# mvrl/RANGE

Measured on AMD Instinct MI355X. Metric: geo-embeddings/sec (10k-query batch, range_db_large), higher is better.
Workload: dtype f32

## Files before the change

### range_amd/csrc/attend_kernels.h

```cpp
#pragma once
#include <hip/hip_runtime.h>
#include <stdint.h>

#include <type_traits>

#include "host_plan.h"

namespace range_hip {

typedef float f32x4 __attribute__((ext_vector_type(4)));

constexpr int KEY_DIM = 256;
constexpr int VAL_DIM = 1024;
constexpr int QTILE = 64;
constexpr int BLK = 16;
constexpr int MAX_TOPK = 16;
constexpr float NEG_BIG = -1.0e30f;

#define RANGE_LPTR(p) ((__attribute__((address_space(3))) void*)(p))

__device__ __forceinline__ int pi_row(int i) { return ((i & 2) << 2) | ((i >> 2) << 1) | (i & 1); }

struct ScanArgs {
    const float* keys;
// ... 307 lines not shown
            if (a.rowmax)
                smax = fmaxf(smax, fmaxf(fmaxf(ok[0] ? ss[0] : -INFINITY, ok[1] ? ss[1] : -INFINITY),
                                         fmaxf(ok[2] ? ss[2] : -INFINITY, ok[3] ? ss[3] : -INFINITY)));
#pragma unroll
            for (int r = 0; r < 4; ++r) {
                const float p1 = __builtin_amdgcn_exp2f(fmaf(ss[r], a.k_sem, nm1));
                l1 += ok[r] ? p1 : 0.f;
                if (GEO) {
                    const float p2 = __builtin_amdgcn_exp2f(fmaf(sg[r], a.k_geo, nm2));
                    l2 += ok[r] ? p2 : 0.f;
                }
            }
        };
        if (n_here == BLK) tile_stats(std::false_type{});
        else tile_stats(std::true_type{});
        slot ^= 1;
    }
#pragma unroll
    for (int off = 16; off <= 32; off <<= 1) {
        l1 += __shfl_xor(l1, off);
        if (GEO) l2 += __shfl_xor(l2, off);
    }
    const float m1 = a.k_sem;
    float m2 = a.k_geo;
    if (!GEO) { m2 = NEG_BIG; l2 = 0.f; }
    if (q < a.B) {
        if (a.rowmax) a.rowmax[((int64_t)split * a.B + q) * 4 + g] = smax;
        if (g == 0) {
            f32x4 o = {m1, l1, m2, l2};
            *reinterpret_cast<f32x4*>(a.out + ((int64_t)split * a.B + q) * 4) = o;
        }
        if (TOPK) {
            const int64_t base = (((int64_t)split * a.B + q) * 4 + g) * MAX_TOPK;
#pragma unroll
            for (int k = 0; k < MAX_TOPK; ++k) {
                a.cand_val[base + k] = tk.v[TOPK ? k : 0];
                a.cand_idx[base + k] = tk.i[TOPK ? k : 0];
            }
        }
    }
}

__device__ __forceinline__ unsigned long long topk_key(float v, uint32_t row) {
    const uint32_t b = __float_as_uint(v);
    const uint32_t o = (b & 0x80000000u) ? ~b : (b | 0x80000000u);
    return ((unsigned long long)o << 32) | (unsigned long long)(0xFFFFFFFFu - row);
}
__device__ __forceinline__ float topk_key_val(unsigned long long k) {
    const uint32_t o = (uint32_t)(k >> 32);
    return __uint_as_float((o & 0x80000000u) ? (o & 0x7FFFFFFFu) : ~o);
}
__device__ __forceinline__ uint32_t topk_key_row(unsigned long long k) { return 0xFFFFFFFFu - (uint32_t)k; }

struct KeyList {
    unsigned long long k[MAX_TOPK];
    __device__ __forceinline__ void init() {
#pragma unroll
        for (int i = 0; i < MAX_TOPK; ++i) k[i] = 0ull;
    }
    __device__ __forceinline__ void push(unsigned long long x) {
        if (x > k[MAX_TOPK - 1]) {
            k[MAX_TOPK - 1] = x;
#pragma unroll
            for (int i = MAX_TOPK - 1; i > 0; --i) {
                const unsigned long long a = k[i - 1], b = k[i];
                k[i - 1] = a > b ? a : b;
                k[i] = a > b ? b : a;
            }
        }
    }
    __device__ __forceinline__ void pop() {
#pragma unroll
        for (int i = 0; i + 1 < MAX_TOPK; ++i) k[i] = k[i + 1];
        k[MAX_TOPK - 1] = 0ull;
    }
};

typedef uint32_t range_u32x2 __attribute__((ext_vector_type(2)));
__device__ __forceinline__ uint32_t lane_xor16(uint32_t x) {
    const range_u32x2 r = __builtin_amdgcn_permlane16_swap(x, x, false, false);
    return (__lane_id() & 16) ? r[0] : r[1];
}
__device__ __forceinline__ uint32_t lane_xor32(uint32_t x) {
    const range_u32x2 r = __builtin_amdgcn_permlane32_swap(x, x, false, false);
    return (__lane_id() & 32) ? r[0] : r[1];
}
__device__ __forceinline__ float lane_xor16(float x) { return __uint_as_float(lane_xor16(__float_as_uint(x))); }
__device__ __forceinline__ float lane_xor32(float x) { return __uint_as_float(lane_xor32(__float_as_uint(x))); }

__device__ __forceinline__ unsigned long long shfl_xor_u64(unsigned long long x, int m) {
    const uint32_t lo = __shfl_xor((uint32_t)x, m), hi = __shfl_xor((uint32_t)(x >> 32), m);
    return ((unsigned long long)hi << 32) | lo;
}
template <int M>
__device__ __forceinline__ unsigned long long lane_xor_u64(unsigned long long x) {
    static_assert(M == 16 || M == 32, "row swaps exist for lane ^ 16 and lane ^ 32");
    const uint32_t lo = M == 16 ? lane_xor16((uint32_t)x) : lane_xor32((uint32_t)x);
    const uint32_t hi = M == 16 ? lane_xor16((uint32_t)(x >> 32)) : lane_xor32((uint32_t)(x >> 32));
    return ((unsigned long long)hi << 32) | lo;
}

__device__ __forceinline__ void merge_lane_groups(KeyList& L) {
    KeyList R;
#pragma unroll
    for (int i = 0; i < MAX_TOPK; ++i) {
        const unsigned long long h = L.k[0];
        unsigned long long m = h;
        unsigned long long o = lane_xor_u64<16>(m); m = o > m ? o : m;
        o = lane_xor_u64<32>(m); m = o > m ? o : m;
        R.k[i] = m;
        if (h == m && m != 0ull) L.pop();
    }
    L = R;
}

__device__ __forceinline__ void merge_wave(KeyList& L) {
    KeyList R;
#pragma unroll
    for (int i = 0; i < MAX_TOPK; ++i) {
        const unsigned long long h = L.k[0];
        unsigned long long m = h;
#pragma unroll
        for (int off = 1; off < 64; off <<= 1) {
            const unsigned long long o = shfl_xor_u64(m, off);
            m = o > m ? o : m;
        }
        R.k[i] = m;
        if (h == m && m != 0ull) L.pop();
    }
    L = R;
}

__global__ __launch_bounds__(256) void topk_threshold_kernel(const float* __restrict__ rowmax,
                                                             int n_parts, int64_t B,
                                                             float* __restrict__ theta) {
    const int lane = threadIdx.x & 63;
    const int64_t q = (int64_t)blockIdx.x * 4 + (threadIdx.x >> 6);
    if (q >= B) return;
    KeyList L;
    L.init();
    const int total = n_parts * 4;
    for (int e = lane; e < total; e += 64) {
        const float v = rowmax[((int64_t)(e >> 2) * B + q) * 4 + (e & 3)];
        if (v > -INFINITY) L.push(topk_key(v, (uint32_t)e));
    }
    merge_wave(L);
    if (lane == 0) theta[q] = L.k[MAX_TOPK - 1] ? topk_key_val(L.k[MAX_TOPK - 1]) : -INFINITY;
}

__global__ __launch_bounds__(256) void topk_from_logits_kernel(const float* __restrict__ logits,
                                                               int32_t n_blocks, int64_t B,
                                                               int64_t n_valid, int32_t n_chunks,
                                                               const float* __restrict__ theta,
                                                               float* __restrict__ cval,
                                                               int32_t* __restrict__ cidx) {
    const int lane = threadIdx.x & 63, g = lane >> 4;
    const int64_t slot = (int64_t)blockIdx.x * 4 + (threadIdx.x >> 6);
    const int64_t n_slots = (B + 15) / 16;
    if (slot >= n_slots) return;
    const int chunk = blockIdx.y;
    const int b0 = (int)(((int64_t)chunk * n_blocks) / n_chunks);
    const int b1 = (int)(((int64_t)(chunk + 1) * n_blocks) / n_chunks);
    const float* base = logits + ((slot >> 2) * (int64_t)n_blocks * 4 + (slot & 3)) * 256 + 4 * lane;
    int prow[4];
#pragma unroll
    for (int r = 0; r < 4; ++r) prow[r] = pi_row(4 * g + r);
    KeyList L;
    L.init();
    const int64_t qq = slot * 16 + (lane & 15);
    const float th = theta[qq < B ? qq : B - 1];
    constexpr int UNROLL = 8;
    for (int b = b0; b < b1; b += UNROLL) {
        f32x4 v[UNROLL];
#pragma unroll
        for (int u = 0; u < UNROLL; ++u) {
            const int bb = b + u < b1 ? b + u : b1 - 1;
            v[u] = *reinterpret_cast<const f32x4*>(base + (int64_t)bb * 1024);
        }
#pragma unroll
        for (int u = 0; u < UNROLL; ++u) {
            if (b + u < b1) {
                const int64_t row0 = (int64_t)(b + u) * BLK;
#pragma unroll
                for (int r = 0; r < 4; ++r) {
                    const int64_t row = row0 + prow[r];
                    if (v[u][r] >= th && row < n_valid) L.push(topk_key(v[u][r], (uint32_t)row));
                }
            }
        }
    }
    merge_lane_groups(L);
    const int64_t q = slot * 16 + (lane & 15);
    if (g == 0 && q < B) {
        float* ov = cval + ((int64_t)chunk * B + q) * MAX_TOPK;
        int32_t* oi = cidx + ((int64_t)chunk * B + q) * MAX_TOPK;
#pragma unroll
        for (int i = 0; i < MAX_TOPK; ++i) {
            const unsigned long long mm = L.k[i];
            ov[i] = mm ? topk_key_val(mm) : -INFINITY;
            oi[i] = mm ? (int32_t)topk_key_row(mm) : 0x7fffffff;
        }
    }
}

__global__ __launch_bounds__(256) void merge_topk_wave_kernel(const float* __restrict__ cval,
                                                              const int32_t* __restrict__ cidx,
                                                              int n_parts, int64_t B, int per_part,
                                                              int k, int64_t row_offset,
                                                              float* __restrict__ oval,
                                                              int64_t* __restrict__ oidx) {
    const int lane = threadIdx.x & 63;
    const int64_t q = (int64_t)blockIdx.x * 4 + (threadIdx.x >> 6);
    if (q >= B) return;
    KeyList L;
    L.init();
    const int total = n_parts * per_part;
    for (int e = lane; e < total; e += 64) {
        const int p = e / per_part, c = e - p * per_part;
        const int64_t at = ((int64_t)p * B + q) * per_part + c;
        const int32_t row = cidx[at];
        if (row != 0x7fffffff) L.push(topk_key(cval[at], (uint32_t)row));
    }
    merge_wave(L);
    if (lane == 0) {
#pragma unroll
        for (int i = 0; i < MAX_TOPK; ++i) {
            if (i < k) {
                const unsigned long long mm = L.k[i];
                oval[q * k + i] = mm ? topk_key_val(mm) : -INFINITY;
                oidx[q * k + i] = mm ? (int64_t)topk_key_row(mm) + row_offset : (int64_t)-1;
            }
        }
    }
}

__global__ void merge_stats_kernel(const float* parts, int n_parts, int64_t B, float* out) {
    const int64_t q = (int64_t)blockIdx.x * blockDim.x + threadIdx.x;
    if (q >= B) return;
    float m1 = NEG_BIG, l1 = 0.f, m2 = NEG_BIG, l2 = 0.f;
    for (int p = 0; p < n_parts; ++p) {
        const f32x4 s = *reinterpret_cast<const f32x4*>(parts + ((int64_t)p * B + q) * 4);
        merge_ml(m1, l1, s.x, s.y);
        merge_ml(m2, l2, s.z, s.w);
    }
    f32x4 o = {m1, l1, m2, l2};
    *reinterpret_cast<f32x4*>(out + q * 4) = o;
}

__global__ __launch_bounds__(256) void merge_stats_wave_kernel(const float* __restrict__ parts,
                                                               int n_parts, int64_t B,
                                                               float* __restrict__ out) {
    const int lane = threadIdx.x & 63;
    const int64_t q = (int64_t)blockIdx.x * 4 + (threadIdx.x >> 6);
    if (q >= B) return;
    float m1 = NEG_BIG, l1 = 0.f, m2 = NEG_BIG, l2 = 0.f;
    for (int p = lane; p < n_parts; p += 64) {
        const f32x4 s = *reinterpret_cast<const f32x4*>(parts + ((int64_t)p * B + q) * 4);
        merge_ml(m1, l1, s.x, s.y);
        merge_ml(m2, l2, s.z, s.w);
    }
#pragma unroll
    for (int off = 1; off < 64; off <<= 1) {
        merge_ml(m1, l1, __shfl_xor(m1, off), __shfl_xor(l1, off));
        merge_ml(m2, l2, __shfl_xor(m2, off), __shfl_xor(l2, off));
    }
    if (lane == 0) {
        f32x4 o = {m1, l1, m2, l2};
        *reinterpret_cast<f32x4*>(out + q * 4) = o;
    }
}

__global__ void merge_topk_kernel(const float* cval, const int32_t* cidx32, const int64_t* cidx64,
                                  int n_parts, int64_t B, int per_part, int k, int64_t row_offset,
                                  float* oval, int64_t* oidx) {
    const int64_t q = (int64_t)blockIdx.x * blockDim.x + threadIdx.x;
    if (q >= B) return;
    float bv[MAX_TOPK];
    int64_t bi[MAX_TOPK];
    for (int j = 0; j < MAX_TOPK; ++j) { bv[j] = -INFINITY; bi[j] = INT64_MAX; }
    for (int p = 0; p < n_parts; ++p) {
        const int64_t base = ((int64_t)p * B + q) * per_part;
        for (int c = 0; c < per_part; ++c) {
            const float v = cval[base + c];
            const int64_t i = cidx32 ? (cidx32[base + c] == 0x7fffffff
                                            ? INT64_MAX : (int64_t)cidx32[base + c] + row_offset)
                                     : cidx64[base + c];
            if (i == INT64_MAX) continue;
            if (v > bv[k - 1] || (v == bv[k - 1] && i < bi[k - 1])) {
                int j = k - 1;
                while (j > 0 && (v > bv[j - 1] || (v == bv[j - 1] && i < bi[j - 1]))) {
                    bv[j] = bv[j - 1]; bi[j] = bi[j - 1]; --j;
                }
                bv[j] = v; bi[j] = i;
            }
        }
    }
    for (int j = 0; j < k; ++j) { oval[q * k + j] = bv[j]; oidx[q * k + j] = bi[j] == INT64_MAX ? -1 : bi[j]; }
}

__device__ __forceinline__ void mfma_a(f32x4& acc, float a, float b) {
    asm volatile("v_mfma_f32_16x16x4_f32 %0, %1, %2, %0\n\ts_nop 1" : "+a"(acc) : "v"(a), "v"(b));
}

struct PvCarry {
    f32x4 v0a, v1a, v0b, v1b;
    float w0, w1;
};

struct PvOps { f32x4 v0, v1; };

__device__ __forceinline__ void pv_first_reads(const float* vslot, int lane, PvOps& s0, PvOps& s1) {
    const float* base = vslot + (2 * (lane >> 4)) * VAL_DIM + 4 * (lane & 15);
    s0.v0 = *reinterpret_cast<const f32x4*>(base);
    s0.v1 = *reinterpret_cast<const f32x4*>(base + VAL_DIM);
    s1.v0 = *reinterpret_cast<const f32x4*>(base + 64);
    s1.v1 = *reinterpret_cast<const f32x4*>(base + VAL_DIM + 64);
}

__device__ __forceinline__ void pv_exec_carry(f32x4 (&acc)[64], const PvCarry& c) {
    mfma_a(acc[56], c.w0, c.v0a.x);
    mfma_a(acc[57], c.w0, c.v0a.y);
    mfma_a(acc[58], c.w0, c.v0a.z);
    mfma_a(acc[59], c.w0, c.v0a.w);
    mfma_a(acc[56], c.w1, c.v1a.x);
    mfma_a(acc[57], c.w1, c.v1a.y);
    mfma_a(acc[58], c.w1, c.v1a.z);
    mfma_a(acc[59], c.w1, c.v1a.w);
    mfma_a(acc[60], c.w0, c.v0b.x);
    mfma_a(acc[61], c.w0, c.v0b.y);
    mfma_a(acc[62], c.w0, c.v0b.z);
    mfma_a(acc[63], c.w0, c.v0b.w);
    mfma_a(acc[60], c.w1, c.v1b.x);
    mfma_a(acc[61], c.w1, c.v1b.y);
    mfma_a(acc[62], c.w1, c.v1b.z);
    mfma_a(acc[63], c.w1, c.v1b.w);
}

#define RANGE_PV_MFMA(tile, w, v, h)                 \
    mfma_a(acc[tile], w, v);                         \
    __builtin_amdgcn_sched_barrier(0);               \
    hook(h);                                         \
    __builtin_amdgcn_sched_barrier(0)

template <class Hook>
__device__ __forceinline__ void pv_steps(const float* vslot, float w0, float w1, PvOps s0, PvOps s1,
                                         f32x4 (&acc)[64], int lane, PvCarry& carry, Hook&& hook) {
    const float* base = vslot + (2 * (lane >> 4)) * VAL_DIM + 4 * (lane & 15);
    f32x4 v0 = s0.v0, v1 = s0.v1, n0 = s1.v0, n1 = s1.v1;
#pragma unroll
    for (int T = 0; T < 14; ++T) {
        const f32x4 m0 = *reinterpret_cast<const f32x4*>(base + 64 * (T + 2));
        const f32x4 m1 = *reinterpret_cast<const f32x4*>(base + VAL_DIM + 64 * (T + 2));
        RANGE_PV_MFMA(4 * T + 0, w0, v0.x, 8 * T + 0);
        RANGE_PV_MFMA(4 * T + 1, w0, v0.y, 8 * T + 1);
        RANGE_PV_MFMA(4 * T + 2, w0, v0.z, 8 * T + 2);
        RANGE_PV_MFMA(4 * T + 3, w0, v0.w, 8 * T + 3);
        RANGE_PV_MFMA(4 * T + 0, w1, v1.x, 8 * T + 4);
        RANGE_PV_MFMA(4 * T + 1, w1, v1.y, 8 * T + 5);
        RANGE_PV_MFMA(4 * T + 2, w1, v1.z, 8 * T + 6);
        RANGE_PV_MFMA(4 * T + 3, w1, v1.w, 8 * T + 7);
        v0 = n0; v1 = n1; n0 = m0; n1 = m1;
    }
    carry.v0a = v0; carry.v1a = v1; carry.v0b = n0; carry.v1b = n1; carry.w0 = w0; carry.w1 = w1;
}
#undef RANGE_PV_MFMA

__device__ __forceinline__ void acc_fence(f32x4 (&acc)[64]) {
    asm volatile("s_nop 15\n\ts_nop 7" ::: "memory");
#pragma unroll
    for (int i = 0; i < 64; i += 16)
        asm volatile("" : "+a"(acc[i]), "+a"(acc[i + 1]), "+a"(acc[i + 2]), "+a"(acc[i + 3]),
                          "+a"(acc[i + 4]), "+a"(acc[i + 5]), "+a"(acc[i + 6]), "+a"(acc[i + 7]),
                          "+a"(acc[i + 8]), "+a"(acc[i + 9]), "+a"(acc[i + 10]), "+a"(acc[i + 11]),
                          "+a"(acc[i + 12]), "+a"(acc[i + 13]), "+a"(acc[i + 14]), "+a"(acc[i + 15]));
}

struct SegWalk {
    int64_t u, u_end;
    int split, col, cb0, cb;
    __device__ __forceinline__ void init(const ScanArgs& a) {
        col = -1;
        u = u_end = 0;
        cb0 = 0;
        cb = a.n_blocks;
        split = 0;
        if (a.sk_groups == 0) {
            int qt;
            decode_block(a, split, qt);
            const int b0 = (int)(((int64_t)split * a.n_blocks) / a.n_splits);
            const int b1 = (int)(((int64_t)(split + 1) * a.n_blocks) / a.n_splits);
            u = (int64_t)qt * a.n_blocks + b0;
            u_end = u + (b1 - b0);
        }
    }
    __device__ __forceinline__ bool next(const ScanArgs& a, int& qt, int& b0, int& b1, float*& out_tile) {
        if (a.sk_groups == 0) {
            if (u >= u_end) return false;
            qt = (int)(u / a.n_blocks);
            b0 = (int)(u - (int64_t)qt * a.n_blocks);
            b1 = b0 + (int)(u_end - u);
            out_tile = a.out + ((int64_t)split * a.B + (int64_t)qt * QTILE) * VAL_DIM;
            u = u_end;
            return true;
        }
        while (u >= u_end) {
            if (++col >= a.sk_cols) return false;
            cb0 = sk_col_begin(col, a.n_blocks, a.sk_cols);
            cb = sk_col_begin(col + 1, a.n_blocks, a.sk_cols) - cb0;
            const int64_t U = (int64_t)a.n_qtiles * cb;
            u = sk_start(blockIdx.x, U, a.sk_groups);
            u_end = sk_start((int64_t)blockIdx.x + 1, U, a.sk_groups);
        }
        qt = (int)(u / cb);
        const int bo = (int)(u - (int64_t)qt * cb);
        const int64_t left = u_end - u;
        const int n = left < (int64_t)(cb - bo) ? (int)left : cb - bo;
        b0 = cb0 + bo;
        b1 = b0 + n;
        out_tile = a.out + ((int64_t)col * (a.sk_groups + a.n_qtiles) + blockIdx.x + qt) * (QTILE * VAL_DIM);
        u += n;
        return true;
    }
};

constexpr int ATTEND_LDS_BYTES = (3 * 8 * VAL_DIM + 2 * BLK * KEY_DIM + 2 * 64) * 4;
constexpr int P1_WG_PER_CU = 4;
constexpr int SCAN_LDS_BYTES = (2 * BLK * KEY_DIM + 2 * 64) * 4;

template <bool GEO, bool DIAG = false>
__global__ __launch_bounds__(256, 1) void attend_kernel(ScanArgs a) {
    extern __shared__ __attribute__((aligned(16))) char smem[];
    float* vring = reinterpret_cast<float*>(smem);

    const uint32_t lds0 = (uint32_t)(uintptr_t)RANGE_LPTR(smem);
    const uint32_t vring_lds = lds0;
    const uint32_t kring_lds = lds0 + 3 * 8 * VAL_DIM * 4;
    const uint32_t xring_lds = kring_lds + 2 * BLK * KEY_DIM * 4;
    constexpr uint32_t VS_BYTES = 8 * VAL_DIM * 4, KT_BYTES = BLK * KEY_DIM * 4;

    const int lane = threadIdx.x & 63;
    const int wave = __builtin_amdgcn_readfirstlane(threadIdx.x >> 6);
    const int g = lane >> 4;
    const int swz = lane ^ (4 * wave);
    SegWalk walk;
    walk.init(a);
    int qt, b0, b1;
    float* out_tile;
    for (bool first_seg = true; walk.next(a, qt, b0, b1, out_tile); first_seg = false) {
    if (!first_seg) __syncthreads();
    const int nb = b1 - b0;
    const int64_t q = (int64_t)qt * QTILE + wave * 16 + (lane & 15);

    QFrag f;
    load_qfrag(f, a.ehat, a.xq, a.B, q, g);
    float ca, cb, m1, m2;
    {
        const f32x4 st = *reinterpret_cast<const f32x4*>(a.stats + (q < a.B ? q : a.B - 1) * 4);
        m1 = st.x; m2 = st.z;
        ca = a.beta / st.y;
        cb = GEO ? (1.0f - a.beta) / st.w : 0.f;
    }
    pin_qfrag(f);
    asm volatile("" : "+v"(ca), "+v"(cb), "+v"(m1), "+v"(m2));

    f32x4 acc[64];
#pragma unroll
    for (int i = 0; i < 64; ++i) acc[i] = f32x4{0.f, 0.f, 0.f, 0.f};

    KAddr kaddr;
    kaddr.init(lane);
    const char* kring_b = smem + 3 * 8 * VAL_DIM * 4;
    const char* xring_b = kring_b + 2 * BLK * KEY_DIM * 4;
    int prow[4];
    uint32_t kvoff[4];
#pragma unroll
    for (int r = 0; r < 4; ++r) {
        prow[r] = pi_row(4 * g + r);
        kvoff[r] = (uint32_t)((swz ^ r) << 4);
    }
    const int n_left = (int)(a.n_valid - (int64_t)b0 * BLK);

    f32x4 w_cur = {0.f, 0.f, 0.f, 0.f};
    if (nb > 0) {
        const int64_t r0 = (int64_t)b0 * BLK;
        const int64_t r1 = (int64_t)(nb > 1 ? b0 + 1 : b0) * BLK;
        issue_k_tile(a.keys, a.xyz4, r0, kring_lds, xring_lds, wave, lane, swz);
        issue_v_half(a.values, r0, vring_lds, wave, lane);
        issue_v_half(a.values, r0 + 8, vring_lds + VS_BYTES, wave, lane);
        issue_k_tile(a.keys, a.xyz4, r1, kring_lds + KT_BYTES, xring_lds + 256, wave, lane, swz);
        RANGE_WAIT_BARRIER(21);
        QKAcc c;
        qk_mfma<GEO>(kring_b, qk_first_reads<GEO>(kring_b, xring_b, kaddr), kaddr, f, c,
                     [](int) __attribute__((always_inline)) {});
        c.fence();
#pragma unroll
        for (int r = 0; r < 4; ++r) {
            float wr = ca * __builtin_amdgcn_exp2f(fmaf(c.sem(r), a.k_sem, -m1));
            if (GEO) wr = fmaf(cb, __builtin_amdgcn_exp2f(fmaf(c.g[r], a.k_geo, -m2)), wr);
            w_cur[r] = prow[r] < n_left ? wr : 0.f;
        }
    }
    int vs = 0;
    PvCarry carry;
    carry.v0a = carry.v1a = carry.v0b = carry.v1b = f32x4{0.f, 0.f, 0.f, 0.f};
    carry.w0 = carry.w1 = 0.f;
    unsigned long long d_vm0 = 0, d_bar0 = 0, d_pv0 = 0, d_vm1 = 0, d_bar1 = 0, d_qk = 0, d_pv1 = 0;
    unsigned long long d_mark = 0;
    const unsigned long long d_start = DIAG ? stamp() : 0;
    const int b_last = b1 - 1;
    for (int t = 0; t < nb; ++t) {
        const int vs1 = vs == 2 ? 0 : vs + 1;
        const int vs2 = vs1 == 2 ? 0 : vs1 + 1;
        const int bn1 = min(b0 + t + 1, b_last), bn2 = min(b0 + t + 2, b_last);
        const float* vsrc1 = a.values + ((int64_t)bn1 * BLK + 2 * wave) * VAL_DIM;
        const float* ksrc2 = a.keys + ((int64_t)bn2 * BLK + 4 * wave) * KEY_DIM;
        const float* xsrc2 = a.xyz4 + (int64_t)bn2 * BLK * 4;
        const uint32_t vdst_e = vring_lds + vs2 * VS_BYTES + wave * 8192;
        const uint32_t vdst_o = vring_lds + vs * VS_BYTES + wave * 8192;
        const uint32_t kdst = kring_lds + (t & 1) * KT_BYTES + wave * 4096;
        const uint32_t xdst = xring_lds + (t & 1) * 256;
        const uint32_t vvoff = (uint32_t)(lane << 4);
        RANGE_WB(13, d_vm0, d_bar0);
        if (DIAG) d_mark = stamp();
        {
            PvOps s0, s1;
            pv_first_reads(vring + vs * 8 * VAL_DIM, lane, s0, s1);
            pv_exec_carry(acc, carry);
            pv_steps(vring + vs * 8 * VAL_DIM, w_cur[0], w_cur[1], s0, s1, acc, lane, carry,
                     [&](int h) __attribute__((always_inline)) {
                         if (h % 14 == 3) {
                             const int ii = h / 14;
                             if ((ii & 3) == 0) dma_group_begin(vdst_e + (ii >> 2) * 4096);
                             dma_b128_q(vsrc1 + (ii >> 2) * VAL_DIM, vvoff, ii & 3);
                         }
                     });
        }
        if (DIAG) d_pv0 += stamp() - d_mark;
        RANGE_WB(8, d_vm1, d_bar1);
        if (DIAG) d_mark = stamp();
        QKAcc c;
        PvOps s0, s1;
        {
            const char* kt = kring_b + ((t + 1) & 1) * KT_BYTES;
            const KFirst kf = qk_first_reads<GEO>(kt, xring_b + ((t + 1) & 1) * 256, kaddr);
            pv_exec_carry(acc, carry);
            qk_mfma<GEO>(kt, kf, kaddr, f, c, [&](int s_) __attribute__((always_inline)) {
                if (s_ == 13) pv_first_reads(vring + vs1 * 8 * VAL_DIM, lane, s0, s1);
            });
        }
        if (DIAG) { const unsigned long long x_ = stamp(); d_qk += x_ - d_mark; d_mark = x_; }
        f32x4 w_next = {0.f, 0.f, 0.f, 0.f};
        float e1[4], e2[4];
        const int n_left1 = n_left - (t + 1) * BLK;
        pv_steps(vring + vs1 * 8 * VAL_DIM, w_cur[2], w_cur[3], s0, s1, acc, lane, carry,
                [&](int h) __attribute__((always_inline)) {
                    if ((h & 7) == 3) {
                        const int ii = h >> 3;
                        if (ii < 8) {
                            if ((ii & 3) == 0) dma_group_begin(vdst_o + (ii >> 2) * 4096);
                            dma_b128_q(vsrc1 + (8 + (ii >> 2)) * VAL_DIM, vvoff, ii & 3);
                        } else if (ii < 12) {
                            if (ii == 8) dma_group_begin(kdst);
                            dma_b128_q(ksrc2, kvoff[ii - 8], ii - 8);
                        } else if (ii == 12) {
                            dma_b32(xsrc2, (uint32_t)(lane << 2), xdst);
                        }
                    } else if (h >= 21 && h < 101 && ((h - 21) & 3) == 0) {
                        const int k = (h - 21) >> 2, r = k / 5, part = k % 5;
                        if (part == 0) {
                        } else if (part == 1) {
                            e1[r] = fmaf(c.a0[r], a.k_sem, -m1);
                            if (GEO) e2[r] = fmaf(c.g[r], a.k_geo, -m2);
                        } else if (part == 2) {
                            e1[r] = __builtin_amdgcn_exp2f(e1[r]);
                        } else if (part == 3) {
                            if (GEO) e2[r] = __builtin_amdgcn_exp2f(e2[r]);
                        } else {
                            float wr = ca * e1[r];
                            if (GEO) wr = fmaf(cb, e2[r], wr);
                            w_next[r] = prow[r] < n_left1 ? wr : 0.f;
                        }
                    }
                });
        if (DIAG) d_pv1 += stamp() - d_mark;
        w_cur = w_next;
        vs = vs2;
    }
    if (nb > 0) pv_exec_carry(acc, carry);
    asm volatile("s_waitcnt vmcnt(0)" ::: "memory");
    if (DIAG && lane == 0 && a.diag) {
        unsigned long long* d = a.diag + ((size_t)blockIdx.x * 4 + wave) * 16;
        d[0] = d_vm0; d[1] = d_bar0; d[2] = d_pv0; d[3] = d_vm1; d[4] = d_bar1; d[5] = d_qk;
        d[6] = d_pv1; d[7] = stamp() - d_start; d[8] = (unsigned long long)nb; d[9] = d_start;
        unsigned xcc; asm volatile("s_getreg_b32 %0, hwreg(HW_REG_XCC_ID)" : "=s"(xcc));
        d[10] = xcc & 0xf;
    }

    acc_fence(acc);
    const int j = lane & 15;
    const int64_t qw = (int64_t)qt * QTILE + wave * 16;
#pragma unroll
    for (int r = 0; r < 4; ++r) {
        const int64_t qo = qw + 4 * g + r;
        if (qo < a.B) {
            float* orow = out_tile + (wave * 16 + 4 * g + r) * VAL_DIM + 4 * j;
#pragma unroll
            for (int T = 0; T < 16; ++T) {
                f32x4 o = {acc[4 * T + 0][r], acc[4 * T + 1][r], acc[4 * T + 2][r], acc[4 * T + 3][r]};
                *reinterpret_cast<f32x4*>(orow + 64 * T) = o;
            }
        }
    }
    }
}

constexpr int ATTEND_STORED_LDS_BYTES = (3 * 8 * VAL_DIM + 2 * 1024 + 2 * 64) * 4;

template <bool GEO>
__global__ __launch_bounds__(256, 1) void attend_stored_kernel(ScanArgs a) {
    extern __shared__ __attribute__((aligned(16))) char smem[];
    float* vring = reinterpret_cast<float*>(smem);
    const uint32_t lds0 = (uint32_t)(uintptr_t)RANGE_LPTR(smem);
    const uint32_t vring_lds = lds0;
    const uint32_t sring_lds = lds0 + 3 * 8 * VAL_DIM * 4;
    const uint32_t xring_lds = sring_lds + 2 * 4096;
    constexpr uint32_t VS_BYTES = 8 * VAL_DIM * 4;

    const int lane = threadIdx.x & 63;
    const int wave = __builtin_amdgcn_readfirstlane(threadIdx.x >> 6);
    const int g = lane >> 4;
    SegWalk walk;
    walk.init(a);
    int qt, b0, b1;
    float* out_tile;
    for (bool first_seg = true; walk.next(a, qt, b0, b1, out_tile); first_seg = false) {
    if (!first_seg) __syncthreads();
    const int nb = b1 - b0;
    const int64_t q = (int64_t)qt * QTILE + wave * 16 + (lane & 15);
    const int64_t qtile_kept = (int64_t)qt + a.qt_offset;

    float ca, cb, m1, m2, fxq;
    {
        const int64_t qq = q < a.B ? q : a.B - 1;
        const f32x4 st = *reinterpret_cast<const f32x4*>(a.stats + qq * 4);
        m1 = st.x; m2 = st.z;
        ca = a.beta / st.y;
        cb = GEO ? (1.0f - a.beta) / st.w : 0.f;
        fxq = a.xq[qq * 4 + g];
    }
    asm volatile("" : "+v"(ca), "+v"(cb), "+v"(m1), "+v"(m2), "+v"(fxq));

    f32x4 acc[64];
#pragma unroll
    for (int i = 0; i < 64; ++i) acc[i] = f32x4{0.f, 0.f, 0.f, 0.f};

    const char* sring_b = smem + 3 * 8 * VAL_DIM * 4;
    const char* xring_b = sring_b + 2 * 4096;
    const uint32_t s_rd = (uint32_t)(wave * 1024 + lane * 16);
    const uint32_t x_rd = (uint32_t)((pi_row(lane & 15) * 4 + g) * 4);
    int prow[4];
#pragma unroll
    for (int r = 0; r < 4; ++r) prow[r] = pi_row(4 * g + r);
    const int n_left = (int)(a.n_valid - (int64_t)b0 * BLK);
    const uint32_t vvoff = (uint32_t)(lane << 4);

    auto issue_sx = [&](int block, int slot) __attribute__((always_inline)) {
        dma_b128(a.logits + logit_tile(qtile_kept, a.n_blocks, block, wave), vvoff,
                 sring_lds + slot * 4096 + wave * 1024);
        dma_b32(a.xyz4 + (int64_t)block * BLK * 4, (uint32_t)(lane << 2), xring_lds + slot * 256);
    };

    f32x4 w_cur = {0.f, 0.f, 0.f, 0.f};
    if (nb > 0) {
        const int64_t r0 = (int64_t)b0 * BLK;
        issue_sx(b0, 0);
        issue_v_half(a.values, r0, vring_lds, wave, lane);
        issue_v_half(a.values, r0 + 8, vring_lds + VS_BYTES, wave, lane);
        issue_sx(nb > 1 ? b0 + 1 : b0, 1);
        RANGE_WAIT_BARRIER(18);
        const f32x4 sv = *reinterpret_cast<const f32x4*>(sring_b + s_rd);
        f32x4 cg = {0.f, 0.f, 0.f, 0.f};
        if (GEO) {
            const float xa = *reinterpret_cast<const float*>(xring_b + x_rd);
            mfma_v_first(cg, xa, fxq);
            asm volatile("s_nop 15" : "+v"(cg));
        }
#pragma unroll
        for (int r = 0; r < 4; ++r) {
            float wr = ca * __builtin_amdgcn_exp2f(fmaf(sv[r], a.k_sem, -m1));
            if (GEO) wr = fmaf(cb, __builtin_amdgcn_exp2f(fmaf(cg[r], a.k_geo, -m2)), wr);
            w_cur[r] = prow[r] < n_left ? wr : 0.f;
        }
    }
    int vs = 0;
    PvCarry carry;
    carry.v0a = carry.v1a = carry.v0b = carry.v1b = f32x4{0.f, 0.f, 0.f, 0.f};
    carry.w0 = carry.w1 = 0.f;
    const int b_last = b1 - 1;
    for (int t = 0; t < nb; ++t) {
        const int vs1 = vs == 2 ? 0 : vs + 1;
        const int vs2 = vs1 == 2 ? 0 : vs1 + 1;
        const int bn1 = min(b0 + t + 1, b_last), bn2 = min(b0 + t + 2, b_last);
        const float* vsrc1 = a.values + ((int64_t)bn1 * BLK + 2 * wave) * VAL_DIM;
        const float* ssrc2 = a.logits + logit_tile(qtile_kept, a.n_blocks, bn2, wave);
        const float* xsrc2 = a.xyz4 + (int64_t)bn2 * BLK * 4;
        const uint32_t vdst_e = vring_lds + vs2 * VS_BYTES + wave * 8192;
        const uint32_t vdst_o = vring_lds + vs * VS_BYTES + wave * 8192;
        const uint32_t sdst = sring_lds + (t & 1) * 4096 + wave * 1024;
        const uint32_t xdst = xring_lds + (t & 1) * 256;
        RANGE_WAIT_BARRIER(10);
        {
            PvOps s0, s1;
            pv_first_reads(vring + vs * 8 * VAL_DIM, lane, s0, s1);
            pv_exec_carry(acc, carry);
            pv_steps(vring + vs * 8 * VAL_DIM, w_cur[0], w_cur[1], s0, s1, acc, lane, carry,
                     [&](int h) __attribute__((always_inline)) {
                         if (h % 14 == 3) {
                             const int ii = h / 14;
                             if ((ii & 3) == 0) dma_group_begin(vdst_e + (ii >> 2) * 4096);
                             dma_b128_q(vsrc1 + (ii >> 2) * VAL_DIM, vvoff, ii & 3);
                         }
                     });
        }
        RANGE_WAIT_BARRIER(8);
        PvOps s0, s1;
        f32x4 cg = {0.f, 0.f, 0.f, 0.f};
        const f32x4 sv = *reinterpret_cast<const f32x4*>(sring_b + ((t + 1) & 1) * 4096 + s_rd);
        {
            const float xa = GEO ? *reinterpret_cast<const float*>(xring_b + ((t + 1) & 1) * 256 + x_rd) : 0.f;
            pv_first_reads(vring + vs1 * 8 * VAL_DIM, lane, s0, s1);
            pv_exec_carry(acc, carry);
            if (GEO) mfma_v_first(cg, xa, fxq);
        }
        f32x4 w_next = {0.f, 0.f, 0.f, 0.f};
        float e1[4], e2[4];
        const int n_left1 = n_left - (t + 1) * BLK;
        pv_steps(vring + vs1 * 8 * VAL_DIM, w_cur[2], w_cur[3], s0, s1, acc, lane, carry,
                [&](int h) __attribute__((always_inline)) {
                    if ((h & 7) == 3) {
                        const int ii = h >> 3;
                        if (ii < 8) {
                            if ((ii & 3) == 0) dma_group_begin(vdst_o + (ii >> 2) * 4096);
                            dma_b128_q(vsrc1 + (8 + (ii >> 2)) * VAL_DIM, vvoff, ii & 3);
                        } else if (ii == 8) {
                            dma_b128(ssrc2, vvoff, sdst);
                        } else if (ii == 9) {
                            dma_b32(xsrc2, (uint32_t)(lane << 2), xdst);
                        }
                    } else if (h >= 22 && h < 78 && (h & 1) == 0) {
                        const int k = (h - 22) >> 1, r = k / 7, op = k % 7;
                        if (op == 0) e1[r] = fmaf(sv[r], a.k_sem, -m1);
                        else if (op == 1) { if (GEO) e2[r] = fmaf(cg[r], a.k_geo, -m2); }
                        else if (op == 2) e1[r] = __builtin_amdgcn_exp2f(e1[r]);
                        else if (op == 3) { if (GEO) e2[r] = __builtin_amdgcn_exp2f(e2[r]); }
                        else if (op == 4) e1[r] = ca * e1[r];
                        else if (op == 5) { if (GEO) e1[r] = fmaf(cb, e2[r], e1[r]); }
                        else w_next[r] = e1[r];
                    }
                });
        if (n_left1 < BLK) {
#pragma unroll
            for (int r = 0; r < 4; ++r) w_next[r] = prow[r] < n_left1 ? w_next[r] : 0.f;
        }
        w_cur = w_next;
        vs = vs2;
    }
    if (nb > 0) pv_exec_carry(acc, carry);
    asm volatile("s_waitcnt vmcnt(0)" ::: "memory");

    acc_fence(acc);
    const int j = lane & 15;
    const int64_t qw = (int64_t)qt * QTILE + wave * 16;
#pragma unroll
    for (int r = 0; r < 4; ++r) {
        const int64_t qo = qw + 4 * g + r;
        if (qo < a.B) {
            float* orow = out_tile + (wave * 16 + 4 * g + r) * VAL_DIM + 4 * j;
#pragma unroll
            for (int T = 0; T < 16; ++T) {
                f32x4 o = {acc[4 * T + 0][r], acc[4 * T + 1][r], acc[4 * T + 2][r], acc[4 * T + 3][r]};
                *reinterpret_cast<f32x4*>(orow + 64 * T) = o;
            }
        }
    }
    }
}


__global__ void reduce_parts_kernel(const float* parts, SlabMap m, int64_t B, float* out) {
    const int64_t i = (int64_t)blockIdx.x * blockDim.x + threadIdx.x;
    if (i >= B * (VAL_DIM / 4)) return;
    const int64_t q = i / (VAL_DIM / 4);
    const int c4 = (int)(i - q * (VAL_DIM / 4));
    f32x4 s = {0.f, 0.f, 0.f, 0.f};
    for (int col = 0; col < slab_cols(m); ++col) {
        int64_t first4, stride4;
        int n;
        slab_parts(m, B, q, col, first4, stride4, n);
        const f32x4* p4 = reinterpret_cast<const f32x4*>(parts) + first4 + c4;
        if (col == 0) s = p4[0];
#pragma unroll 4
        for (int p = col == 0 ? 1 : 0; p < n; ++p) s += p4[(int64_t)p * stride4];
    }
    reinterpret_cast<f32x4*>(out)[i] = s;
}

__global__ void blend_kernel(const float* G, const float* H, float beta, int64_t n4, float* out) {
    const int64_t i = (int64_t)blockIdx.x * blockDim.x + threadIdx.x;
    if (i >= n4) return;
    const f32x4 g = reinterpret_cast<const f32x4*>(G)[i];
    const f32x4 h = reinterpret_cast<const f32x4*>(H)[i];
    const float a = 1.0f - beta;
    f32x4 o;
#pragma unroll
    for (int k = 0; k < 4; ++k) o[k] = __fadd_rn(__fmul_rn(a, g[k]), __fmul_rn(beta, h[k]));
    reinterpret_cast<f32x4*>(out)[i] = o;
}

__global__ void finalize_kernel(const float* parts, SlabMap m, const double* ehat64, int64_t B,
                                int64_t q0, int64_t nq, double* out) {
    const int64_t i = (int64_t)blockIdx.x * blockDim.x + threadIdx.x;
    if (i >= nq * 320) return;
    const int64_t q = q0 + i / 320;
    const int c = (int)(i % 320);
    double* o = out + q * 1280 + 4 * c;
    if (c < 256) {
        f32x4 s = {0.f, 0.f, 0.f, 0.f};
        for (int col = 0; col < slab_cols(m); ++col) {
            int64_t first4, stride4;
            int n;
            slab_parts(m, B, q, col, first4, stride4, n);
            const f32x4* p4 = reinterpret_cast<const f32x4*>(parts) + first4 + c;
            if (col == 0) s = p4[0];
#pragma unroll 8
            for (int p = col == 0 ? 1 : 0; p < n; ++p) s += p4[(int64_t)p * stride4];
        }
        o[0] = (double)s.x; o[1] = (double)s.y; o[2] = (double)s.z; o[3] = (double)s.w;
    } else {
        const double* e = ehat64 + q * 256 + 4 * (c - 256);
        o[0] = e[0]; o[1] = e[1]; o[2] = e[2]; o[3] = e[3];
    }
}

}
```

Measured before the change: 521,700.

## Restructure stored-attend pipeline to full-block double buffering with one barrier per block

Replaces the three-slot half-block value ring with two full 16-row value buffers, so each block is processed in one 128-step MFMA sweep behind a single wait/barrier instead of two half-block phases. The loop is unrolled by two with compile-time parity so buffer offsets are constants, and the DMA issue for the next block's logits, coords and values is spread across the first 128 hook slots. The softmax weight computation moves later in the sweep. Tail padding is now applied only to the final block. The aim is to halve barriers and cut address arithmetic, at the cost of more LDS use and a longer prefetch distance per barrier.

Result: faster. 527,000 (median of 6 runs) (+1.0%).

```diff
diff --git a/range_amd/csrc/attend_kernels.h b/range_amd/csrc/attend_kernels.h
--- a/range_amd/csrc/attend_kernels.h
+++ b/range_amd/csrc/attend_kernels.h
@@ -633,6 +633,17 @@
     asm volatile("v_mfma_f32_16x16x4_f32 %0, %1, %2, %0\n\ts_nop 1" : "+a"(acc) : "v"(a), "v"(b));
 }
 
+__device__ __forceinline__ float valu_mul(float a, float b) {
+    float d;
+    asm volatile("v_mul_f32 %0, %1, %2" : "=v"(d) : "v"(a), "v"(b));
+    return d;
+}
+__device__ __forceinline__ float valu_fma(float a, float b, float c) {
+    float d;
+    asm volatile("v_fma_f32 %0, %1, %2, %3" : "=v"(d) : "v"(a), "v"(b), "v"(c));
+    return d;
+}
+
 struct PvCarry {
     f32x4 v0a, v1a, v0b, v1b;
     float w0, w1;
@@ -696,6 +707,43 @@
 }
 #undef RANGE_PV_MFMA
 
+template <int S, class Hook>
+__device__ __forceinline__ void pv_block_step(const float* base, const f32x4& w, f32x4& v0, f32x4& v1,
+                                              f32x4& n0, f32x4& n1, f32x4 (&acc)[64], Hook& hook) {
+#define RANGE_PV_MFMA(tile, w, v, h)                 \
+    mfma_a(acc[tile], w, v);                         \
+    __builtin_amdgcn_sched_barrier(0);               \
+    hook(h);                                         \
+    __builtin_amdgcn_sched_barrier(0)
+    if constexpr (S < 30) {
+        constexpr int T = S & 15, S2 = S + 2;
+        const float* src = base + (S2 >> 4) * 8 * VAL_DIM + 64 * (S2 & 15);
+        const f32x4 m0 = *reinterpret_cast<const f32x4*>(src);
+        const f32x4 m1 = *reinterpret_cast<const f32x4*>(src + VAL_DIM);
+        const float w0 = S < 16 ? w[0] : w[2], w1 = S < 16 ? w[1] : w[3];
+        RANGE_PV_MFMA(4 * T + 0, w0, v0.x, 8 * S + 0);
+        RANGE_PV_MFMA(4 * T + 1, w0, v0.y, 8 * S + 1);
+        RANGE_PV_MFMA(4 * T + 2, w0, v0.z, 8 * S + 2);
+        RANGE_PV_MFMA(4 * T + 3, w0, v0.w, 8 * S + 3);
+        RANGE_PV_MFMA(4 * T + 0, w1, v1.x, 8 * S + 4);
+        RANGE_PV_MFMA(4 * T + 1, w1, v1.y, 8 * S + 5);
+        RANGE_PV_MFMA(4 * T + 2, w1, v1.z, 8 * S + 6);
+        RANGE_PV_MFMA(4 * T + 3, w1, v1.w, 8 * S + 7);
+        v0 = n0; v1 = n1; n0 = m0; n1 = m1;
+        pv_block_step<S + 1>(base, w, v0, v1, n0, n1, acc, hook);
+    }
+#undef RANGE_PV_MFMA
+}
+
+template <class Hook>
+__device__ __forceinline__ void pv_block_steps(const float* vslot, const f32x4& w, PvOps s0, PvOps s1,
+                                               f32x4 (&acc)[64], int lane, PvCarry& carry, Hook&& hook) {
+    const float* base = vslot + (2 * (lane >> 4)) * VAL_DIM + 4 * (lane & 15);
+    f32x4 v0 = s0.v0, v1 = s0.v1, n0 = s1.v0, n1 = s1.v1;
+    pv_block_step<0>(base, w, v0, v1, n0, n1, acc, hook);
+    carry.v0a = v0; carry.v1a = v1; carry.v0b = n0; carry.v1b = n1; carry.w0 = w[2]; carry.w1 = w[3];
+}
+
 __device__ __forceinline__ void acc_fence(f32x4 (&acc)[64]) {
     asm volatile("s_nop 15\n\ts_nop 7" ::: "memory");
 #pragma unroll
@@ -704,6 +752,13 @@
                           "+a"(acc[i + 4]), "+a"(acc[i + 5]), "+a"(acc[i + 6]), "+a"(acc[i + 7]),
                           "+a"(acc[i + 8]), "+a"(acc[i + 9]), "+a"(acc[i + 10]), "+a"(acc[i + 11]),
                           "+a"(acc[i + 12]), "+a"(acc[i + 13]), "+a"(acc[i + 14]), "+a"(acc[i + 15]));
+}
+
+__device__ __forceinline__ void carry_wait_states() { asm volatile("s_nop 1"); }
+
+__device__ __forceinline__ void acc_pin(f32x4 (&acc)[64]) {
+#pragma unroll
+    for (int i = 0; i < 64; ++i) asm volatile("" : "+a"(acc[i]));
 }
 
 struct SegWalk {
@@ -945,17 +1000,19 @@
     }
 }
 
-constexpr int ATTEND_STORED_LDS_BYTES = (3 * 8 * VAL_DIM + 2 * 1024 + 2 * 64) * 4;
+constexpr int ATTEND_STORED_LDS_BYTES = (2 * BLK * VAL_DIM + 2 * 1024 + 2 * 64) * 4;
+
+template <int V> struct IntC { __device__ constexpr operator int() const { return V; } };
 
 template <bool GEO>
 __global__ __launch_bounds__(256, 1) void attend_stored_kernel(ScanArgs a) {
     extern __shared__ __attribute__((aligned(16))) char smem[];
     float* vring = reinterpret_cast<float*>(smem);
+    constexpr uint32_t VB_BYTES = BLK * VAL_DIM * 4;
     const uint32_t lds0 = (uint32_t)(uintptr_t)RANGE_LPTR(smem);
     const uint32_t vring_lds = lds0;
-    const uint32_t sring_lds = lds0 + 3 * 8 * VAL_DIM * 4;
+    const uint32_t sring_lds = lds0 + 2 * VB_BYTES;
     const uint32_t xring_lds = sring_lds + 2 * 4096;
-    constexpr uint32_t VS_BYTES = 8 * VAL_DIM * 4;
 
     const int lane = threadIdx.x & 63;
     const int wave = __builtin_amdgcn_readfirstlane(threadIdx.x >> 6);
@@ -984,8 +1041,9 @@
     f32x4 acc[64];
 #pragma unroll
     for (int i = 0; i < 64; ++i) acc[i] = f32x4{0.f, 0.f, 0.f, 0.f};
-
-    const char* sring_b = smem + 3 * 8 * VAL_DIM * 4;
+    acc_pin(acc);
+
+    const char* sring_b = smem + 2 * VB_BYTES;
     const char* xring_b = sring_b + 2 * 4096;
     const uint32_t s_rd = (uint32_t)(wave * 1024 + lane * 16);
     const uint32_t x_rd = (uint32_t)((pi_row(lane & 15) * 4 + g) * 4);
@@ -1000,13 +1058,17 @@
                  sring_lds + slot * 4096 + wave * 1024);
         dma_b32(a.xyz4 + (int64_t)block * BLK * 4, (uint32_t)(lane << 2), xring_lds + slot * 256);
     };
-
-    f32x4 w_cur = {0.f, 0.f, 0.f, 0.f};
+    auto zero_pad_rows = [&](f32x4& w, int valid) __attribute__((always_inline)) {
+#pragma unroll
+        for (int r = 0; r < 4; ++r) w[r] = prow[r] < valid ? w[r] : 0.f;
+    };
+
+    f32x4 w_a = {0.f, 0.f, 0.f, 0.f}, w_b = {0.f, 0.f, 0.f, 0.f};
     if (nb > 0) {
         const int64_t r0 = (int64_t)b0 * BLK;
         issue_sx(b0, 0);
         issue_v_half(a.values, r0, vring_lds, wave, lane);
-        issue_v_half(a.values, r0 + 8, vring_lds + VS_BYTES, wave, lane);
+        issue_v_half(a.values, r0 + 8, vring_lds + VB_BYTES / 2, wave, lane);
         issue_sx(nb > 1 ? b0 + 1 : b0, 1);
         RANGE_WAIT_BARRIER(18);
         const f32x4 sv = *reinterpret_cast<const f32x4*>(sring_b + s_rd);
@@ -1020,83 +1082,79 @@
         for (int r = 0; r < 4; ++r) {
             float wr = ca * __builtin_amdgcn_exp2f(fmaf(sv[r], a.k_sem, -m1));
             if (GEO) wr = fmaf(cb, __builtin_amdgcn_exp2f(fmaf(cg[r], a.k_geo, -m2)), wr);
-            w_cur[r] = prow[r] < n_left ? wr : 0.f;
-        }
-    }
-    int vs = 0;
+            w_a[r] = wr;
+        }
+    }
     PvCarry carry;
     carry.v0a = carry.v1a = carry.v0b = carry.v1b = f32x4{0.f, 0.f, 0.f, 0.f};
     carry.w0 = carry.w1 = 0.f;
     const int b_last = b1 - 1;
-    for (int t = 0; t < nb; ++t) {
-        const int vs1 = vs == 2 ? 0 : vs + 1;
-        const int vs2 = vs1 == 2 ? 0 : vs1 + 1;
+
+    auto run_block = [&](auto par, int t, const f32x4& w_cur, f32x4& w_next) __attribute__((always_inline)) {
+        const int P = par;
         const int bn1 = min(b0 + t + 1, b_last), bn2 = min(b0 + t + 2, b_last);
         const float* vsrc1 = a.values + ((int64_t)bn1 * BLK + 2 * wave) * VAL_DIM;
         const float* ssrc2 = a.logits + logit_tile(qtile_kept, a.n_blocks, bn2, wave);
         const float* xsrc2 = a.xyz4 + (int64_t)bn2 * BLK * 4;
-        const uint32_t vdst_e = vring_lds + vs2 * VS_BYTES + wave * 8192;
-        const uint32_t vdst_o = vring_lds + vs * VS_BYTES + wave * 8192;
-        const uint32_t sdst = sring_lds + (t & 1) * 4096 + wave * 1024;
-        const uint32_t xdst = xring_lds + (t & 1) * 256;
-        RANGE_WAIT_BARRIER(10);
-        {
-            PvOps s0, s1;
-            pv_first_reads(vring + vs * 8 * VAL_DIM, lane, s0, s1);
-            pv_exec_carry(acc, carry);
-            pv_steps(vring + vs * 8 * VAL_DIM, w_cur[0], w_cur[1], s0, s1, acc, lane, carry,
-                     [&](int h) __attribute__((always_inline)) {
-                         if (h % 14 == 3) {
-                             const int ii = h / 14;
-                             if ((ii & 3) == 0) dma_group_begin(vdst_e + (ii >> 2) * 4096);
-                             dma_b128_q(vsrc1 + (ii >> 2) * VAL_DIM, vvoff, ii & 3);
-                         }
-                     });
-        }
-        RANGE_WAIT_BARRIER(8);
+        const uint32_t vdst = vring_lds + (P ^ 1) * VB_BYTES + wave * 8192;
+        const uint32_t sdst = sring_lds + P * 4096 + wave * 1024;
+        const uint32_t xdst = xring_lds + P * 256;
+        const float* vslot = vring + P * BLK * VAL_DIM;
+        RANGE_WAIT_BARRIER(0);
         PvOps s0, s1;
         f32x4 cg = {0.f, 0.f, 0.f, 0.f};
-        const f32x4 sv = *reinterpret_cast<const f32x4*>(sring_b + ((t + 1) & 1) * 4096 + s_rd);
+        const f32x4 sv = *reinterpret_cast<const f32x4*>(sring_b + (P ^ 1) * 4096 + s_rd);
         {
-            const float xa = GEO ? *reinterpret_cast<const float*>(xring_b + ((t + 1) & 1) * 256 + x_rd) : 0.f;
-            pv_first_reads(vring + vs1 * 8 * VAL_DIM, lane, s0, s1);
+            const float xa = GEO ? *reinterpret_cast<const float*>(xring_b + (P ^ 1) * 256 + x_rd) : 0.f;
+            pv_first_reads(vslot, lane, s0, s1);
+            carry_wait_states();
             pv_exec_carry(acc, carry);
             if (GEO) mfma_v_first(cg, xa, fxq);
         }
-        f32x4 w_next = {0.f, 0.f, 0.f, 0.f};
         float e1[4], e2[4];
-        const int n_left1 = n_left - (t + 1) * BLK;
-        pv_steps(vring + vs1 * 8 * VAL_DIM, w_cur[2], w_cur[3], s0, s1, acc, lane, carry,
+        pv_block_steps(vslot, w_cur, s0, s1, acc, lane, carry,
                 [&](int h) __attribute__((always_inline)) {
-                    if ((h & 7) == 3) {
-                        const int ii = h >> 3;
-                        if (ii < 8) {
-                            if ((ii & 3) == 0) dma_group_begin(vdst_o + (ii >> 2) * 4096);
-                            dma_b128_q(vsrc1 + (8 + (ii >> 2)) * VAL_DIM, vvoff, ii & 3);
-                        } else if (ii == 8) {
-                            dma_b128(ssrc2, vvoff, sdst);
-                        } else if (ii == 9) {
-                            dma_b32(xsrc2, (uint32_t)(lane << 2), xdst);
+                    if (h < 128) {
+                        if (h % 6 == 3) {
+                            const int ii = h / 6;
+                            if (ii == 0) {
+                                dma_b128(ssrc2, vvoff, sdst);
+                            } else if (ii == 1) {
+                                dma_b32(xsrc2, (uint32_t)(lane << 2), xdst);
+                            } else if (ii < 18) {
+                                const int p = ii - 2, hh = p >> 3, row = (p >> 2) & 1, qq = p & 3;
+                                if (qq == 0) dma_group_begin(vdst + hh * (VB_BYTES / 2) + row * 4096);
+                                dma_b128_q(vsrc1 + (8 * hh + row) * VAL_DIM, vvoff, qq);
+                            }
                         }
-                    } else if (h >= 22 && h < 78 && (h & 1) == 0) {
-                        const int k = (h - 22) >> 1, r = k / 7, op = k % 7;
+                    } else if (h >= 150 && h < 206 && (h & 1) == 0) {
+                        const int k = (h - 150) >> 1, r = k / 7, op = k % 7;
                         if (op == 0) e1[r] = fmaf(sv[r], a.k_sem, -m1);
                         else if (op == 1) { if (GEO) e2[r] = fmaf(cg[r], a.k_geo, -m2); }
                         else if (op == 2) e1[r] = __builtin_amdgcn_exp2f(e1[r]);
                         else if (op == 3) { if (GEO) e2[r] = __builtin_amdgcn_exp2f(e2[r]); }
-                        else if (op == 4) e1[r] = ca * e1[r];
-                        else if (op == 5) { if (GEO) e1[r] = fmaf(cb, e2[r], e1[r]); }
+                        else if (op == 4) e1[r] = valu_mul(ca, e1[r]);
+                        else if (op == 5) { if (GEO) e1[r] = valu_fma(cb, e2[r], e1[r]); }
                         else w_next[r] = e1[r];
                     }
                 });
-        if (n_left1 < BLK) {
-#pragma unroll
-            for (int r = 0; r < 4; ++r) w_next[r] = prow[r] < n_left1 ? w_next[r] : 0.f;
-        }
-        w_cur = w_next;
-        vs = vs2;
-    }
-    if (nb > 0) pv_exec_carry(acc, carry);
+    };
+
+    if (nb > 0) {
+        const int valid_last = n_left - (nb - 1) * BLK;
+        int t = 0;
+        for (; t + 2 <= nb; t += 2) {
+            run_block(IntC<0>{}, t, w_a, w_b);
+            if (t + 2 == nb && valid_last < BLK) zero_pad_rows(w_b, valid_last);
+            run_block(IntC<1>{}, t + 1, w_b, w_a);
+        }
+        if (t < nb) {
+            if (valid_last < BLK) zero_pad_rows(w_a, valid_last);
+            run_block(IntC<0>{}, t, w_a, w_b);
+        }
+        carry_wait_states();
+        pv_exec_carry(acc, carry);
+    }
     asm volatile("s_waitcnt vmcnt(0)" ::: "memory");
 
     acc_fence(acc);
```
